# OPM/opm-autodiff

Measured on AMD Instinct MI355X. Metric: Newton iterations/sec, 1M-cell 3-phase black-oil (assembly + ILU0/BiCGStab solve + update), higher is better.
Workload: dtype f64

## Files before the change

### opm-autodiff_amd/csrc/internal.hpp

```cpp
#pragma once
#include <hip/hip_runtime.h>

#include <cstdarg>
#include <cstdio>
#include <cstdlib>
#include <cstring>
#include <memory>
#include <climits>
#include <string>
#include <type_traits>
#include <vector>

#include "../../include/opmhip.h"
#include "cpr_setup.hpp"

namespace opmhip {

constexpr int BS = 3;
constexpr int BB = 9;

#ifndef OPMHIP_TILE_ROWS
#define OPMHIP_TILE_ROWS 32
#endif
constexpr int TILE_ROWS = OPMHIP_TILE_ROWS;
// ... 285 lines not shown
    int ilu_fillin = 0;
    opmhip::Pattern pat;
    double *d_A = nullptr, *d_L = nullptr, *d_U = nullptr, *d_invD = nullptr;
    double *d_R = nullptr, *d_usum = nullptr;
    bool half_product = false;
    double *d_b = nullptr, *d_x = nullptr, *d_r = nullptr, *d_rw = nullptr, *d_p = nullptr, *d_v = nullptr,
           *d_s = nullptr, *d_t = nullptr, *d_pw = nullptr, *d_vu = nullptr;
    double *d_stageA = nullptr, *d_stageV = nullptr;
    double* d_scal = nullptr;
    double* d_part = nullptr;
    double minv_scale = 1.0;
    double* d_part2 = nullptr;
    int npart = 0;
    int last_solve_iterations = 0;
    int last_dot_count = 0;
    double* h_pinned = nullptr;
    static constexpr int RB_SLOTS = 4, RB_DOUBLES = 4;
    double* h_ring = nullptr;
    double* d_ring = nullptr;
    double rb_seq = 0.0;
    double rb_want[RB_SLOTS] = {0, 0, 0, 0};
    const double* d_done = nullptr;
    opmhip::WellsDev wells;
    opmhip::AsmDev asmb;
    opmhip::CommDev comm;
    opmhip::CprDev cpr;
    opmhip::Profiler prof;
    std::vector<void*> allocs;
    struct HostRange { const void* p; size_t bytes; };
    std::vector<HostRange> pinned;
// ... 136 lines not shown
    return slot;
}
inline void prof_span_end(opmhip_ctx* c, int slot, hipStream_t s = nullptr) {
    if (slot < 0) return;
    const int e = prof_event(c, s);
    if (e >= 0) c->prof.e1[slot] = e; else c->prof.cls[slot] = -1;
}

int build_pattern(opmhip_ctx* c, int Nb, int Nghost, int nnzb, const int* rows, const int* cols);

void launch_permute_blocks(opmhip_ctx* c, const double* nat, double* internal);
void launch_unpermute_blocks(opmhip_ctx* c, const double* internal, double* nat);
void launch_vec_to_internal(opmhip_ctx* c, const double* nat, double* internal, int cells = -1);
void launch_vec_to_natural(opmhip_ctx* c, const double* internal, double* nat, int cells = -1);
void launch_zero_diag_fix(opmhip_ctx* c);
int launch_spmv(opmhip_ctx* c, double* x, double* y, int ndot, const double* w0, double xs = 1.0, bool exchange = false, const double* uadd = nullptr, const double* w1 = nullptr);
bool half_product_wanted(const opmhip_ctx* c);
void launch_wells_residual(opmhip_ctx* c, const double* d_resWell, double* r);
void launch_wells_add_to_matrix(opmhip_ctx* c, int w0, int nw, int serial, const int* d_pair_ptr, const int* d_entry);
int launch_wells_recover(opmhip_ctx* c, const double* d_resWell, const double* x, double* d_xw);
void launch_ilu_factor(opmhip_ctx* c, bool fix_zero_diagonal = false, const FactorRider* rider = nullptr);
int cpr_factor_rider(opmhip_ctx* c, FactorRider* r);
void launch_ilu_apply(opmhip_ctx* c, const double* d, double* v, double w_override = -1.0, double* unscaled = nullptr, const double* addp = nullptr, double* work = nullptr, double* usum = nullptr);
int cpr_update(opmhip_ctx* c, bool solveBoundary = true);
void launch_cpr_apply(opmhip_ctx* c, const double* d, double* v);
int cpr_set_weights(opmhip_ctx* c, const double* w);
int cpr_level_sizes(const opmhip_ctx* c, int* n, int* nnz, int cap);
void cpr_shutdown(opmhip_ctx* c);
bool cpr_coarse_pivot_failed(opmhip_ctx* c);
int cpr_ilu_levels_in_force(const opmhip_ctx* c);
inline bool use_cpr(const opmhip_ctx* c) { return c->cfg.preconditioner == OPMHIP_PRECOND_CPR_QUASIIMPES || c->cfg.preconditioner == OPMHIP_PRECOND_CPR_TRUEIMPES; }
// ... 41 lines not shown
```

### opm-autodiff_amd/csrc/solver.hip

```cpp
#include <hip/hip_runtime.h>
#include <hip/hip_ext.h>
#include <atomic>

#include <chrono>
#include <cmath>
#include <cstdlib>

#include "internal.hpp"

namespace opmhip {

#ifndef OPMHIP_STAGE_DEPTH
#define OPMHIP_STAGE_DEPTH 16
#endif
typedef double v2d_t __attribute__((ext_vector_type(2)));
__device__ __forceinline__ double2 ld_stream(const double2* p) {
    const v2d_t t = __builtin_nontemporal_load(reinterpret_cast<const v2d_t*>(p));
    return make_double2(t.x, t.y);
}
__device__ __forceinline__ void st_rowsum(double* p, double v) {
    __builtin_nontemporal_store(v, p);
}
__device__ __forceinline__ void stage_doubles(const double* __restrict__ src, double* __restrict__ dst, int n, int lane) {
    const double2* __restrict__ s2 = reinterpret_cast<const double2*>(src);
// ... 267 lines not shown
                             const double* __restrict__ L, const double* __restrict__ U, const double* __restrict__ invD,
                             double* __restrict__ out) {
    const int p = blockIdx.x * blockDim.x + threadIdx.x;
    if (p >= Nb) return;
    int li = lrowptr[p], ui = urowptr[p];
    for (int k = rowptr[p]; k < rowptr[p + 1]; ++k) {
        if (col[k] >= Nb) {
            for (int q = 0; q < BB; ++q) out[(size_t)k * BB + q] = 0.0;
            continue;
        }
        const double* src = (col[k] < p) ? &L[(size_t)(li++) * BB] : (col[k] == p) ? &invD[(size_t)p * BB] : &U[(size_t)(ui++) * BB];
        for (int q = 0; q < BB; ++q) out[(size_t)k * BB + q] = src[q];
    }
}

template <int NDOT>
__global__ __launch_bounds__(64) void k_spmv(const int4* __restrict__ sched, const int* __restrict__ rowptr,
                                             const int* __restrict__ col, const double* __restrict__ val,
                                             const double* __restrict__ x, double* __restrict__ y,
                                             const double* __restrict__ w0, double* __restrict__ part, int npart,
                                             const double* __restrict__ done, double xs) {
    TILE_LDS
    const int lane = threadIdx.x, t = blockIdx.x;
    if (*done != 0.0) return;
    const int4 rows = sched[t];
    if (rows.y <= rows.x) {
        if (NDOT >= 1 && lane == 0) { part[t] = 0.0; if (NDOT == 2) part[npart + t] = 0.0; }
        return;
    }
    TileCtx T;
// ... 155 lines not shown
        __builtin_amdgcn_sched_barrier(0);
    }
    if (NDOT >= 1) {
        sd0 = wave_sum(sd0);
        if (NDOT == 2) sd1 = wave_sum(sd1);
        if (lane == 0) { part[blockIdx.x] = sd0; if (NDOT == 2) part[npart + blockIdx.x] = sd1; }
    }
}

template <int NDOT, bool UADD = false>
__global__ __launch_bounds__(64) void k_spmv_pipe_st(int npos, const int4* __restrict__ sched, const unsigned* __restrict__ stWord,
                                                     const unsigned char* __restrict__ stKoff, const int* __restrict__ stTable,
                                                     const double* __restrict__ val, const double* __restrict__ x, double* __restrict__ y,
                                                     const double* __restrict__ w0, double* __restrict__ part, int npart,
                                                     const double* __restrict__ done, double xs, const double* __restrict__ uadd = nullptr,
                                                     const double* __restrict__ w1 = nullptr) {
    TILE_LDS
    __shared__ int4 ssched[PIPE_MAX_STEPS];
    const int lane = threadIdx.x, G = gridDim.x;
    constexpr int U = 16;
    const int nsteps = ((int)blockIdx.x < npos) ? (npos - (int)blockIdx.x + G - 1) / G : 0;
    if (nsteps <= 0) {
        if (NDOT >= 1 && lane == 0) { part[blockIdx.x] = 0.0; if (NDOT >= 2) part[npart + blockIdx.x] = 0.0; if (NDOT == 3) part[2 * npart + blockIdx.x] = 0.0; }
        return;
    }
    const double stop = *done;
    for (int i = lane; i < nsteps; i += 64) ssched[i] = sched[(int)blockIdx.x + i * G];
    if (stop != 0.0) return;
    wave_sync();
    struct StW { unsigned w; int koff, tab; };
    struct StS {
        int k0e, n, n2;
        double2 tmp[U];
    };
    struct StM {
        int kb, nrow;
        double xx[PGCH][3];
        double ww[NDOT >= 1 ? 3 : 1];
// ... 97 lines not shown
                if (NDOT >= 2) { double d1 = acc[0] * acc[0]; d1 += acc[1] * acc[1]; d1 += acc[2] * acc[2]; sd1 += d1; }
                if constexpr (NDOT == 3) { double d2 = acc[0] * m.w2[0]; d2 += acc[1] * m.w2[1]; d2 += acc[2] * m.w2[2]; sd2 += d2; }
            }
        }
        wave_sync();
        __builtin_amdgcn_sched_barrier(0);
        stageGm(st + 1, wq, m);
        __builtin_amdgcn_sched_barrier(0);
        stageW(st + 2, wq);
        __builtin_amdgcn_sched_barrier(0);
    }
    if (NDOT >= 1) {
        sd0 = wave_sum(sd0);
        if (NDOT >= 2) sd1 = wave_sum(sd1);
        if (NDOT == 3) sd2 = wave_sum(sd2);
        if (lane == 0) { part[blockIdx.x] = sd0; if (NDOT >= 2) part[npart + blockIdx.x] = sd1; if (NDOT == 3) part[2 * npart + blockIdx.x] = sd2; }
    }
}

enum { SW_L = 0, SW_LF = 1, SW_UF = 2 };
template <int K> __device__ __forceinline__ double second_result(const double* __restrict__ addp, int r, double wout) {
    if (!addp) return wout;
    return (K == 1 ? addp[r] : 0.0) + wout;
}
template <int SHAPE>
__global__ __launch_bounds__(64) void k_ilu_sweep(int tile_begin, int ntc, int n0, int rhs_from_d, const int* __restrict__ tile_row0,
                                                  const int* __restrict__ prow, const int* __restrict__ pcol,
                                                  const double* __restrict__ P, const double* __restrict__ invD,
                                                  const double* __restrict__ d, double* __restrict__ vu, double* __restrict__ v,
                                                  const double* __restrict__ addp, int relax_mode, double w, const double* __restrict__ done) {
    TILE_LDS
// ... 844 lines not shown
                for (int k = 0; k < 4; ++k) s += Dw[i * 4 + k] * Bb[k * 3 + j];
                tmp[i][j] = s;
            }
        double* blk = &A[(size_t)entry[pair_ptr[w] + q] * BB];
        for (int i = 0; i < 3; ++i)
            for (int j = 0; j < 3; ++j) {
                double s = 0.0;
                for (int k = 0; k < 4; ++k) s += Cc[k * 3 + i] * tmp[k][j];
                blk[i * 3 + j] += -s;
            }
    }
}

constexpr int VB = 256;
constexpr int VPT = 8;
__device__ __forceinline__ void block_partials(double a, double b, double* part, int npart, int nsum) {
    __shared__ double sh[2][VB / 64];
    a = wave_sum(a);
    if (nsum > 1) b = wave_sum(b);
    const int lane = threadIdx.x & 63, wv = threadIdx.x >> 6;
    if (lane == 0) { sh[0][wv] = a; sh[1][wv] = b; }
    __syncthreads();
    if (threadIdx.x == 0) {
        double s = sh[0][0];
        for (int i = 1; i < VB / 64; ++i) s += sh[0][i];
        part[blockIdx.x] = s;
        if (nsum > 1) {
            double u = sh[1][0];
            for (int i = 1; i < VB / 64; ++i) u += sh[1][i];
            part[npart + blockIdx.x] = u;
        }
    }
}
__global__ __launch_bounds__(VB) void k_bicg_init(int n, const double* __restrict__ b, double* __restrict__ r,
                                                  double* __restrict__ rw, double* __restrict__ p, double* __restrict__ x,
                                                  double* __restrict__ v, double* __restrict__ part, int npart) {
    double s = 0.0;
    const int base = blockIdx.x * VB * VPT + threadIdx.x;
#pragma unroll
    for (int u = 0; u < VPT; ++u) {
        const int e = base + u * VB;
        if (e < n) {
            const double be = b[e];
            r[e] = be; rw[e] = be; p[e] = be; x[e] = 0.0; v[e] = 0.0;
            s += be * be;
        }
    }
    block_partials(s, 0.0, part, npart, 1);
}
__global__ __launch_bounds__(VB) void k_bicg_pupdate(int n, const double* __restrict__ scal, double* __restrict__ p,
                                                     const double* __restrict__ v, const double* __restrict__ r) {
    if (scal[SC_DONE] != 0.0) return;
    const double omega = scal[SC_OMEGA], beta = scal[SC_BETA];
    const int base = blockIdx.x * VB * VPT + threadIdx.x;
#pragma unroll
    for (int u = 0; u < VPT; ++u) {
        const int e = base + u * VB;
        if (e < n) p[e] = (p[e] - omega * __builtin_nontemporal_load(&v[e])) * beta + r[e];
    }
}
template <bool SR = false>
__global__ __launch_bounds__(VB) void k_bicg_upd1(int n, const double* __restrict__ scal, double* __restrict__ r,
                                                  const double* __restrict__ v, double* __restrict__ part, int npart, double half = -1.0) {
    if (scal[SC_DONE] != 0.0 && !(SR && scal[SC_DONEH] == half)) return;
    const double alpha = scal[SC_ALPHA];
    double s = 0.0;
    const int base = blockIdx.x * VB * VPT + threadIdx.x;
#pragma unroll
    for (int u = 0; u < VPT; ++u) {
        const int e = base + u * VB;
        if (e < n) {
            const double re = r[e] - alpha * __builtin_nontemporal_load(&v[e]);
            r[e] = re;
            s += re * re;
        }
    }
    if (!SR) block_partials(s, 0.0, part, npart, 1);
}
__global__ __launch_bounds__(VB) void k_bicg_xhalf(int n, const double* __restrict__ scal, double* __restrict__ x, const double* __restrict__ pw, double ws) {
    const double alpha = scal[SC_ALPHA];
    const int base = blockIdx.x * VB * VPT + threadIdx.x;
#pragma unroll
    for (int u = 0; u < VPT; ++u) {
        const int e = base + u * VB;
        if (e < n) x[e] += alpha * (ws * pw[e]);
    }
}
template <bool SR = false>
__global__ __launch_bounds__(VB) void k_bicg_upd2(int n, const double* __restrict__ scal, double* __restrict__ x,
                                                  const double* __restrict__ pw, const double* __restrict__ sv, double* __restrict__ r,
                                                  const double* __restrict__ tv, const double* __restrict__ rw,
                                                  double* __restrict__ part, int npart, double ws, double half = -1.0) {
    if (scal[SC_DONE] != 0.0 && !(SR && scal[SC_DONEH] == half)) return;
    const double alpha = scal[SC_ALPHA], omega = scal[SC_OMEGA];
    double s = 0.0, q = 0.0;
    const int base = blockIdx.x * VB * VPT + threadIdx.x;
#pragma unroll
    for (int u = 0; u < VPT; ++u) {
        const int e = base + u * VB;
        if (e < n) {
            const double xh = __builtin_nontemporal_load(&x[e]) + alpha * (ws * __builtin_nontemporal_load(&pw[e]));
            __builtin_nontemporal_store(xh + omega * (ws * __builtin_nontemporal_load(&sv[e])), &x[e]);
            const double re = r[e] - omega * __builtin_nontemporal_load(&tv[e]);
            r[e] = re;
            s += re * re;
            q += rw[e] * re;
        }
    }
    if (!SR) block_partials(s, q, part, npart, 2);
}
__global__ __launch_bounds__(VB) void k_dots(int n, const double* __restrict__ a, const double* __restrict__ b,
                                             double* __restrict__ part, int npart, int nsum) {
    double s = 0.0, q = 0.0;
    const int base = blockIdx.x * VB * VPT + threadIdx.x;
#pragma unroll
    for (int u = 0; u < VPT; ++u) {
        const int e = base + u * VB;
        if (e < n) { s += a[e] * b[e]; q += a[e] * a[e]; }
    }
    block_partials(s, q, part, npart, nsum);
}
__global__ __launch_bounds__(VB) void k_dots3(int n, const double* __restrict__ a, const double* __restrict__ b, const double* __restrict__ c3,
                                              double* __restrict__ part, int npart) {
    __shared__ double sh[3][VB / 64];
// ... 55 lines not shown
        case FIN_NORM_RHO: {
            scal[SC_NORM] = sqrt(s0);
            const double rhop = scal[SC_RHO];
            scal[SC_RHOP] = rhop; scal[SC_RHO] = s1;
            scal[SC_BETA] = (s1 / rhop) * (scal[SC_ALPHA] / scal[SC_OMEGA]);
        } break;
    }
    if (hslot && (mode == FIN_NORM || mode == FIN_NORM_RHO)) {
        const double norm = scal[SC_NORM], norm0 = scal[SC_NORM0];
        const double stop = (norm < tol * norm0) ? 1.0 : 0.0;
        scal[SC_DONE] = stop;
        hslot[0] = norm; hslot[1] = norm0; hslot[2] = stop;
        __hip_atomic_store(&hslot[3], seq, __ATOMIC_RELEASE, __HIP_MEMORY_SCOPE_SYSTEM);
    }
}
__device__ __forceinline__ void finalize_scalars3(int mode, double s0, double s1, double s2, double* __restrict__ scal, double tol, double* hslot, double seq, double half) {
    const double rr = scal[SC_RR];
    double rrn;
    if (mode == FIN_SR1) {
        const double rho = scal[SC_RHO];
        const double alpha = rho / s0;
        scal[SC_TMP1] = s0;
        scal[SC_ALPHA] = alpha;
        rrn = (rr - 2.0 * alpha * s2) + alpha * alpha * s1;
        scal[SC_RHOH] = rho - alpha * s0;
    } else {
        const double omega = s0 / s1;
        scal[SC_TMP1] = s0; scal[SC_TMP2] = s1;
        scal[SC_OMEGA] = omega;
        rrn = (rr - 2.0 * omega * s0) + omega * omega * s1;
// ... 51 lines not shown
    finalize_scalars3(mode, a, b, c3, scal, tol, hslot, seq, half);
}
__global__ __launch_bounds__(VB) void k_finalize(int mode, int count, const double* __restrict__ part, int npart,
                                                 double* __restrict__ scal, double tol, double* hslot, double seq) {
    __shared__ double sh[2][VB];
    constexpr int FU = 8;
    double va[FU], vb[FU];
#pragma unroll
    for (int u = 0; u < FU; ++u) {
        const int i = (int)threadIdx.x + u * VB;
        const int j = i < count ? i : 0;
        va[u] = part[j]; vb[u] = part[npart + j];
    }
    const double stop = (mode != FIN_INIT && mode != FIN_TRUE) ? scal[SC_DONE] : 0.0;
    if (stop != 0.0) {
        if (threadIdx.x == 0 && hslot && (mode == FIN_NORM || mode == FIN_NORM_RHO)) {
            hslot[0] = scal[SC_NORM]; hslot[1] = scal[SC_NORM0]; hslot[2] = 1.0;
            __hip_atomic_store(&hslot[3], seq, __ATOMIC_RELEASE, __HIP_MEMORY_SCOPE_SYSTEM);
        }
        return;
    }
    double a = 0.0, b = 0.0;
#pragma unroll
    for (int u = 0; u < FU; ++u)
        if ((int)threadIdx.x + u * VB < count) { a += va[u]; b += vb[u]; }
    for (int i = (int)threadIdx.x + FU * VB; i < count; i += VB) { a += part[i]; b += part[npart + i]; }
    sh[0][threadIdx.x] = a; sh[1][threadIdx.x] = b;
    __syncthreads();
    for (int o = VB / 2; o >= 64; o >>= 1) {
        if ((int)threadIdx.x < o) { sh[0][threadIdx.x] += sh[0][threadIdx.x + o]; sh[1][threadIdx.x] += sh[1][threadIdx.x + o]; }
        __syncthreads();
    }
    if (threadIdx.x >= 64) return;
    a = sh[0][threadIdx.x]; b = sh[1][threadIdx.x];
#pragma unroll
    for (int o = 32; o > 0; o >>= 1) { a += __shfl_down(a, o, 64); b += __shfl_down(b, o, 64); }
    if (threadIdx.x != 0) return;
    finalize_scalars(mode, a, b, scal, tol, hslot, seq);
}
static_assert(RED1_BLOCKS <= VB, "the last workgroup holds one slice sum per thread");
__global__ __launch_bounds__(VB) void k_reduce_finalize(int mode, int count, const double* __restrict__ part, int npart, double* out,
                                                        unsigned* ticket, double* __restrict__ scal, double tol, double* hslot, double seq) {
    __shared__ double sh[2][VB];
    __shared__ bool last;
    if (mode != FIN_INIT && mode != FIN_LOCAL && mode != FIN_TRUE && scal[SC_DONE] != 0.0) {
        if (blockIdx.x == 0 && threadIdx.x == 0 && hslot && (mode == FIN_NORM || mode == FIN_NORM_RHO)) {
            hslot[0] = scal[SC_NORM]; hslot[1] = scal[SC_NORM0]; hslot[2] = 1.0;
            __hip_atomic_store(&hslot[3], seq, __ATOMIC_RELEASE, __HIP_MEMORY_SCOPE_SYSTEM);
        }
        return;
    }
    const int chunk = (count + RED1_BLOCKS - 1) / RED1_BLOCKS;
    const int b0 = blockIdx.x * chunk, e0 = min(count, b0 + chunk);
    double a0 = 0.0, a1 = 0.0;
    for (int i = b0 + threadIdx.x; i < e0; i += VB) { a0 += part[i]; a1 += part[npart + i]; }
    sh[0][threadIdx.x] = a0; sh[1][threadIdx.x] = a1;
    __syncthreads();
    for (int o = VB / 2; o > 0; o >>= 1) {
        if ((int)threadIdx.x < o) { sh[0][threadIdx.x] += sh[0][threadIdx.x + o]; sh[1][threadIdx.x] += sh[1][threadIdx.x + o]; }
        __syncthreads();
    }
    if (threadIdx.x == 0) {
        __hip_atomic_store(&out[blockIdx.x], sh[0][0], __ATOMIC_RELAXED, __HIP_MEMORY_SCOPE_AGENT);
        __hip_atomic_store(&out[RED1_BLOCKS + blockIdx.x], sh[1][0], __ATOMIC_RELAXED, __HIP_MEMORY_SCOPE_AGENT);
// ... 107 lines not shown
    const int w = spmv_pipe_wgs(c);
    return c->pat.maxRowBlocks <= PGCH && w > 0 && c->pat.tiles.nsched > w;
}
bool half_product_wanted(const opmhip_ctx* c) {
    const Pattern& P = c->pat;
    if (!P.rest.on || c->cfg.half_product < 0 || use_cpr(c)) return false;
    if (c->cfg.half_product > 0) return true;
    return spmv_pipelined(c);
}
static bool spmv_dots_env() {
    static const bool v = [] { const char* e = tuning_env("OPMHIP_DOTS_SEPARATE"); return e && std::atoi(e) != 0; }();
    return v;
}
static bool spmv_dots_separate(const opmhip_ctx* c) { return c->wells.any() || spmv_dots_env(); }
static int launch_spmv_part(opmhip_ctx* c, int p0, int np, const double* x, double* y, int ndot, const double* w0, double xs, int pofs, int cls,
                            const double* uadd = nullptr, const double* w1 = nullptr) {
    const Pattern& P = c->pat;
    if (np <= 0) return 0;
    double* part = c->d_part + pofs;
    int es = -1, ee = -1;
    const bool timed = prof_kernel_scope(c, cls, &es, &ee);
    hipEvent_t e0 = timed ? c->prof.ev[es] : nullptr, e1 = timed ? c->prof.ev[ee] : nullptr;
    if (uadd) {
        const RestSched& R = P.rest;
        const int4* rsched = reinterpret_cast<const int4*>(R.d_sched) + p0;
        const int pipeWgs = std::max(8, spmv_pipe_wgs(c));
        const int steps = std::min((np + pipeWgs - 1) / pipeWgs, PIPE_MAX_STEPS);
        const int grid = 8 * (((np + steps - 1) / steps + 7) / 8);
        const int* tab = R.d_table + (size_t)p0 * 16;
        if (ndot == 0)
            hipExtLaunchKernelGGL((k_spmv_pipe_st<0, true>), dim3(grid), dim3(64), 0, c->stream, e0, e1, 0, np, rsched, R.d_word, R.d_koff, tab, c->d_R, x, y, w0, part, c->npart, c->d_done, xs, uadd, (const double*)nullptr);
        else if (ndot == 1)
            hipExtLaunchKernelGGL((k_spmv_pipe_st<1, true>), dim3(grid), dim3(64), 0, c->stream, e0, e1, 0, np, rsched, R.d_word, R.d_koff, tab, c->d_R, x, y, w0, part, c->npart, c->d_done, xs, uadd, (const double*)nullptr);
        else if (ndot == 2)
            hipExtLaunchKernelGGL((k_spmv_pipe_st<2, true>), dim3(grid), dim3(64), 0, c->stream, e0, e1, 0, np, rsched, R.d_word, R.d_koff, tab, c->d_R, x, y, w0, part, c->npart, c->d_done, xs, uadd, (const double*)nullptr);
        else
            hipExtLaunchKernelGGL((k_spmv_pipe_st<3, true>), dim3(grid), dim3(64), 0, c->stream, e0, e1, 0, np, rsched, R.d_word, R.d_koff, tab, c->d_R, x, y, w0, part, c->npart, c->d_done, xs, uadd, w1);
        return ndot > 0 ? grid : 0;
    }
    const int4* sched = reinterpret_cast<const int4*>(P.tiles.d_spmvSched) + p0;
    if (spmv_pipelined(c)) {
        const int pipeWgs = spmv_pipe_wgs(c);
        const int steps = std::min((np + pipeWgs - 1) / pipeWgs, PIPE_MAX_STEPS);
        const int grid = 8 * (((np + steps - 1) / steps + 7) / 8);
        const bool inInt = p0 < P.tiles.nschedInt, inBnd = p0 + np > P.tiles.nschedInt;
        if ((!inInt || P.tiles.stencilPart[0]) && (!inBnd || P.tiles.stencilPart[1])) {
            const StencilForm& S = P.tiles.st;
            const int* tab = S.d_table + (size_t)p0 * 16;
            if (ndot == 0)
                hipExtLaunchKernelGGL((k_spmv_pipe_st<0, false>), dim3(grid), dim3(64), 0, c->stream, e0, e1, 0, np, sched, S.d_word, S.d_koff, tab, c->d_A, x, y, w0, part, c->npart, c->d_done, xs, (const double*)nullptr, (const double*)nullptr);
            else if (ndot == 1)
                hipExtLaunchKernelGGL((k_spmv_pipe_st<1, false>), dim3(grid), dim3(64), 0, c->stream, e0, e1, 0, np, sched, S.d_word, S.d_koff, tab, c->d_A, x, y, w0, part, c->npart, c->d_done, xs, (const double*)nullptr, (const double*)nullptr);
            else if (ndot == 2)
                hipExtLaunchKernelGGL((k_spmv_pipe_st<2, false>), dim3(grid), dim3(64), 0, c->stream, e0, e1, 0, np, sched, S.d_word, S.d_koff, tab, c->d_A, x, y, w0, part, c->npart, c->d_done, xs, (const double*)nullptr, (const double*)nullptr);
            else
                hipExtLaunchKernelGGL((k_spmv_pipe_st<3, false>), dim3(grid), dim3(64), 0, c->stream, e0, e1, 0, np, sched, S.d_word, S.d_koff, tab, c->d_A, x, y, w0, part, c->npart, c->d_done, xs, (const double*)nullptr, w1);
            return ndot > 0 ? grid : 0;
        }
        if (ndot == 0)
            hipExtLaunchKernelGGL(k_spmv_pipe<0>, dim3(grid), dim3(64), 0, c->stream, e0, e1, 0, np, sched, P.d_rowptr, P.d_col, c->d_A, x, y, w0, part, c->npart, c->d_done, xs);
        else if (ndot == 1)
            hipExtLaunchKernelGGL(k_spmv_pipe<1>, dim3(grid), dim3(64), 0, c->stream, e0, e1, 0, np, sched, P.d_rowptr, P.d_col, c->d_A, x, y, w0, part, c->npart, c->d_done, xs);
        else
            hipExtLaunchKernelGGL(k_spmv_pipe<2>, dim3(grid), dim3(64), 0, c->stream, e0, e1, 0, np, sched, P.d_rowptr, P.d_col, c->d_A, x, y, w0, part, c->npart, c->d_done, xs);
        return ndot > 0 ? grid : 0;
    }
    if (ndot == 0)
        hipExtLaunchKernelGGL(k_spmv<0>, dim3(np), dim3(64), 0, c->stream, e0, e1, 0, sched, P.d_rowptr, P.d_col, c->d_A, x, y, w0, part, c->npart, c->d_done, xs);
    else if (ndot == 1)
        hipExtLaunchKernelGGL(k_spmv<1>, dim3(np), dim3(64), 0, c->stream, e0, e1, 0, sched, P.d_rowptr, P.d_col, c->d_A, x, y, w0, part, c->npart, c->d_done, xs);
    else
// ... 4 lines not shown
    WellsDev& W = c->wells;
    const size_t n = (size_t)c->pat.Nb * BS;
    launch_vec_to_natural(c, x, c->d_stageV);
    OPMHIP_HIP(c, hipMemcpyAsync(W.h_x, c->d_stageV, n * sizeof(double), hipMemcpyDeviceToHost, c->stream));
    launch_vec_to_natural(c, y, c->d_stageV);
    OPMHIP_HIP(c, hipMemcpyAsync(W.h_y, c->d_stageV, n * sizeof(double), hipMemcpyDeviceToHost, c->stream));
    OPMHIP_HIP(c, hipStreamSynchronize(c->stream));
    if (xs != 1.0)
        for (size_t i = 0; i < n; ++i) W.h_x[i] *= xs;
    W.ms_apply(W.ms_user, W.h_x, W.h_y);
    OPMHIP_HIP(c, hipMemcpyAsync(c->d_stageV, W.h_y, n * sizeof(double), hipMemcpyHostToDevice, c->stream));
    launch_vec_to_internal(c, c->d_stageV, y);
    OPMHIP_HIP(c, hipStreamSynchronize(c->stream));
    return OPMHIP_SUCCESS;
}
int launch_spmv(opmhip_ctx* c, double* x, double* y, int ndot, const double* w0, double xs, bool exchange, const double* uadd, const double* w1) {
    const Pattern& P = c->pat;
    const bool wells = c->wells.num_wells > 0;
    const bool bndPlain = uadd && P.Nghost > 0 && P.tiles.nsched > P.tiles.nschedInt;
    const bool plain3 = spmv_pipelined(c);
    const bool rides3 = uadd ? (!bndPlain || (plain3 && P.tiles.stencilPart[1]))
                             : (plain3 && P.tiles.stencilPart[0] && (P.tiles.nsched == P.tiles.nschedInt || P.tiles.stencilPart[1]));
    const int fused = (spmv_dots_separate(c) || (ndot == 3 && !rides3)) ? 0 : ndot;
    const bool halo = exchange && c->comm.halo_set && c->comm.nneigh > 0;
    if (exchange && !halo && c->comm.nranks > 1) comm_halo_bystander(c);
    const int nInt = uadd ? P.rest.nschedInt : P.tiles.nschedInt;
    const int bnd0 = (uadd && !bndPlain) ? P.rest.nschedInt : P.tiles.nschedInt;
    const int nBnd = (uadd && !bndPlain) ? P.rest.nsched - P.rest.nschedInt : P.tiles.nsched - P.tiles.nschedInt;
    const double* uBnd = bndPlain ? nullptr : uadd;
    int rc, cnt = 0;
    if (halo && nBnd > 0) {
        if ((rc = comm_halo_begin(c, x))) return rc;
        cnt += launch_spmv_part(c, 0, nInt, x, y, fused, w0, xs, cnt, PROF_SPMV, uadd, w1);
        if ((rc = comm_halo_end(c))) return rc;
        cnt += launch_spmv_part(c, bnd0, nBnd, x, y, fused, w0, xs, cnt, PROF_SPMV_BOUNDARY, uBnd, w1);
    } else {
        if (halo && (rc = comm_halo_f64(c, x, BS))) return rc;
        cnt += launch_spmv_part(c, 0, nInt, x, y, fused, w0, xs, cnt, PROF_SPMV, uadd, w1);
        if (nBnd > 0) cnt += launch_spmv_part(c, bnd0, nBnd, x, y, fused, w0, xs, cnt, bndPlain ? PROF_SPMV_BOUNDARY : PROF_SPMV, uBnd, w1);
    }
    if (c->wells.num_ms > 0 && (rc = ms_wells_apply(c, x, y, xs))) return rc;
    if (wells && (rc = launch_wells_apply(c, x, y, xs))) return rc;
    if (fused == 0 && ndot > 0) {
        const int n = P.Nb * BS;
        const int ps = prof_begin(c, PROF_VECTOR);
        if (ndot == 3) {
            cnt = std::min(vec_blocks(n), RED1_SINGLE_MAX);
            hipLaunchKernelGGL(k_dots3, dim3(cnt), dim3(VB), 0, c->stream, n, y, w0, w1, c->d_part, c->npart);
        } else {
            hipLaunchKernelGGL(k_dots, dim3(vec_blocks(n)), dim3(VB), 0, c->stream, n, y, w0, c->d_part, c->npart, ndot);
            cnt = vec_blocks(n);
        }
        prof_end(c, ps);
// ... 110 lines not shown
        if (col < C - 1)
            hipLaunchKernelGGL(k_ilu_sweep<SW_L>, grid(nt), dim3(64), 0, c->stream, tb, nt, n0, 0, T.d_row0, P.d_lrowptr, P.d_lcol, c->d_L,
                               c->d_invD, d, vu, v, addp, mode, w, c->d_done);
        else
            hipLaunchKernelGGL(k_ilu_sweep<SW_LF>, grid(nt), dim3(64), 0, c->stream, tb, nt, n0, 0, T.d_row0, P.d_lrowptr, P.d_lcol, c->d_L,
                               c->d_invD, d, vu, v, addp, mode, w, c->d_done);
    }
    for (int col = (C > 1 ? C - 2 : 0); col >= 0; --col) {
        const int tb = T.colorTile[col], nt = T.colorTile[col + 1] - tb;
        if (nt <= 0) continue;
        hipLaunchKernelGGL(k_ilu_sweep<SW_UF>, grid(nt), dim3(64), 0, c->stream, tb, nt, 0, col == 0 ? 1 : 0, T.d_row0, P.d_urowptr, P.d_ucol,
                           c->d_U, c->d_invD, d, vu, v, addp, mode, w, c->d_done);
    }
    prof_end(c, ps);
}
static int finalize(opmhip_ctx* c, int mode, int count, int rb_half = -1) {
    const double tol = c->cfg.tolerance;
    double* hslot = nullptr;
    double seq = 0.0;
    if (rb_half >= 0) {
        const int sl = rb_half % opmhip_ctx::RB_SLOTS;
        hslot = c->d_ring + (size_t)sl * opmhip_ctx::RB_DOUBLES;
        seq = (c->rb_seq += 1.0);
        c->rb_want[sl] = seq;
    }
    if (c->comm.nranks > 1) {
        const int span = prof_span_begin(c, PROF_ALLREDUCE);
        if (count > RED1_SINGLE_MAX)
            hipLaunchKernelGGL(k_reduce_finalize, dim3(RED1_BLOCKS), dim3(VB), 0, c->stream, (int)FIN_LOCAL, count, c->d_part, c->npart, c->d_part2,
                               reinterpret_cast<unsigned*>(c->d_part2 + 2 * RED1_BLOCKS), c->comm.d_red, tol, (double*)nullptr, 0.0);
        else
            hipLaunchKernelGGL(k_local_sums, dim3(1), dim3(VB), 0, c->stream, count, c->d_part, c->npart, c->comm.d_red);
        c->comm.reduce_span_open = true;
        const int rc = comm_allreduce(c, c->comm.d_red, 2, 0);
        c->comm.reduce_span_open = false;
        prof_span_end(c, span);
        if (rc) return rc;
        hipLaunchKernelGGL(k_finalize, dim3(1), dim3(VB), 0, c->stream, mode, 1, c->comm.d_red, 1, c->d_scal, tol, hslot, seq);
        return OPMHIP_SUCCESS;
    }
// ... 34 lines not shown
    (void)finalize(c, FIN_NORM_RHO, nb);
}

static int read_scalars(opmhip_ctx* c) {
    OPMHIP_HIP(c, hipMemcpyAsync(c->h_pinned, c->d_scal, SC_COUNT * sizeof(double), hipMemcpyDeviceToHost, c->stream));
    OPMHIP_HIP(c, hipStreamSynchronize(c->stream));
    return OPMHIP_SUCCESS;
}
enum { HALF_ALL = 0, HALF_PRECOND = 1, HALF_REST = 2 };
static int enqueue_half(opmhip_ctx* c, int h, int part = HALF_ALL) {
    const Pattern& P = c->pat;
    const int n = P.Nb * BS, nb = vec_blocks(n);
    const bool cpr = use_cpr(c);
    const bool hp = !cpr && c->half_product;
    const bool sr = c->cfg.fused_reductions > 0;
    const bool precTalks = cpr && c->cpr.gather.on;
    const bool head = part != HALF_REST, rest = part != HALF_PRECOND;
    const bool applyNow = part == HALF_ALL || (precTalks ? part == HALF_REST : part == HALF_PRECOND);
    int rc, ps;
    if ((h & 1) == 0) {
        if (head && h > 0) {
            ps = prof_begin(c, PROF_VECTOR);
            hipLaunchKernelGGL(k_bicg_pupdate, dim3(nb), dim3(VB), 0, c->stream, n, c->d_scal, c->d_p, c->d_v, c->d_r);
            prof_end(c, ps);
        }
        if (applyNow) {
            if (cpr) launch_cpr_apply(c, c->d_p, c->d_pw);
            else launch_ilu_apply(c, c->d_p, c->d_pw, -1.0, &c->minv_scale, nullptr, nullptr, hp ? c->d_usum : nullptr);
            if (cpr && c->cpr.apply_rc) { rc = c->cpr.apply_rc; c->cpr.apply_rc = 0; return rc; }
        }
        if (!rest) return OPMHIP_SUCCESS;
        if (sr) {
            if ((rc = launch_spmv(c, c->d_pw, c->d_v, 3, c->d_rw, c->minv_scale, true, hp ? c->d_usum : nullptr, c->d_r))) return rc;
            ps = prof_begin(c, PROF_VECTOR);
            if ((rc = finalize3(c, FIN_SR1, dot_count(c), h))) return rc;
            hipLaunchKernelGGL(k_bicg_upd1<true>, dim3(nb), dim3(VB), 0, c->stream, n, c->d_scal, c->d_r, c->d_v, c->d_part, c->npart, (double)h);
            prof_end(c, ps);
            return OPMHIP_SUCCESS;
        }
        if ((rc = launch_spmv(c, c->d_pw, c->d_v, 1, c->d_rw, c->minv_scale, true, hp ? c->d_usum : nullptr))) return rc;
        ps = prof_begin(c, PROF_VECTOR);
        if ((rc = finalize(c, FIN_ALPHA, dot_count(c)))) return rc;
        hipLaunchKernelGGL(k_bicg_upd1<false>, dim3(nb), dim3(VB), 0, c->stream, n, c->d_scal, c->d_r, c->d_v, c->d_part, c->npart, -1.0);
        if ((rc = finalize(c, FIN_NORM, nb, h))) return rc;
        prof_end(c, ps);
    } else {
        if (applyNow) {
            if (cpr) launch_cpr_apply(c, c->d_r, c->d_s);
            else launch_ilu_apply(c, c->d_r, c->d_s, -1.0, &c->minv_scale, nullptr, nullptr, hp ? c->d_usum : nullptr);
            if (cpr && c->cpr.apply_rc) { rc = c->cpr.apply_rc; c->cpr.apply_rc = 0; return rc; }
        }
        if (!rest) return OPMHIP_SUCCESS;
        if (sr) {
            if ((rc = launch_spmv(c, c->d_s, c->d_t, 3, c->d_r, c->minv_scale, true, hp ? c->d_usum : nullptr, c->d_rw))) return rc;
            ps = prof_begin(c, PROF_VECTOR);
            if ((rc = finalize3(c, FIN_SR2, dot_count(c), h))) return rc;
            hipLaunchKernelGGL(k_bicg_upd2<true>, dim3(nb), dim3(VB), 0, c->stream, n, c->d_scal, c->d_x, c->d_pw, c->d_s, c->d_r, c->d_t, c->d_rw, c->d_part, c->npart, c->minv_scale, (double)h);
            prof_end(c, ps);
            return OPMHIP_SUCCESS;
        }
        if ((rc = launch_spmv(c, c->d_s, c->d_t, 2, c->d_r, c->minv_scale, true, hp ? c->d_usum : nullptr))) return rc;
        ps = prof_begin(c, PROF_VECTOR);
        if ((rc = finalize(c, FIN_OMEGA, dot_count(c)))) return rc;
        hipLaunchKernelGGL(k_bicg_upd2<false>, dim3(nb), dim3(VB), 0, c->stream, n, c->d_scal, c->d_x, c->d_pw, c->d_s, c->d_r, c->d_t, c->d_rw, c->d_part, c->npart, c->minv_scale, -1.0);
        if ((rc = finalize(c, FIN_NORM_RHO, nb, h))) return rc;
        prof_end(c, ps);
    }
    return OPMHIP_SUCCESS;
}
static int wait_half(opmhip_ctx* c, int h, double* norm, double* norm_0) {
    const int sl = h % opmhip_ctx::RB_SLOTS;
    const volatile double* slot = c->h_ring + (size_t)sl * opmhip_ctx::RB_DOUBLES;
    const double want = c->rb_want[sl];
    const auto t0 = std::chrono::steady_clock::now();
    for (unsigned long spin = 1;; ++spin) {
        if (slot[3] == want) break;
        if ((spin & 0xFFFFu) == 0) {
            const hipError_t e = hipStreamQuery(c->stream);
            if (e == hipSuccess) {
                if (slot[3] == want) break;
// ... 89 lines not shown
```

Baseline: 81.23.

## Fold BiCGStab scalar finalize into last-block of SpMV and update kernels

Adds a last-workgroup ticket scheme so the final block of the SpMV dot-product kernel and the vector-update kernels reduces the per-block partials and computes the BiCGStab scalars (alpha, omega, norm/rho) itself. This removes separate finalize kernel launches from each half iteration, cutting launch count and serialization on the stream. In exchange it adds agent-scope atomic stores, a global ticket counter, and a serial single-wave reduction at the tail of each kernel. It only runs on single-rank, half-product, non-fused-reduction paths without wells or boundary rows, and an environment variable can turn it off.

```diff
diff --git a/opm-autodiff_amd/csrc/internal.hpp b/opm-autodiff_amd/csrc/internal.hpp
--- a/opm-autodiff_amd/csrc/internal.hpp
+++ b/opm-autodiff_amd/csrc/internal.hpp
@@ -323,6 +323,7 @@
     int npart = 0;
     int last_solve_iterations = 0;
     int last_dot_count = 0;
+    bool last_dots_folded = false;
     double* h_pinned = nullptr;
     static constexpr int RB_SLOTS = 4, RB_DOUBLES = 4;
     double* h_ring = nullptr;
@@ -489,7 +490,9 @@
 void launch_vec_to_internal(opmhip_ctx* c, const double* nat, double* internal, int cells = -1);
 void launch_vec_to_natural(opmhip_ctx* c, const double* internal, double* nat, int cells = -1);
 void launch_zero_diag_fix(opmhip_ctx* c);
-int launch_spmv(opmhip_ctx* c, double* x, double* y, int ndot, const double* w0, double xs = 1.0, bool exchange = false, const double* uadd = nullptr, const double* w1 = nullptr);
+struct FinFold;
+int launch_spmv(opmhip_ctx* c, double* x, double* y, int ndot, const double* w0, double xs = 1.0, bool exchange = false, const double* uadd = nullptr, const double* w1 = nullptr,
+                const FinFold* fin = nullptr);
 bool half_product_wanted(const opmhip_ctx* c);
 void launch_wells_residual(opmhip_ctx* c, const double* d_resWell, double* r);
 void launch_wells_add_to_matrix(opmhip_ctx* c, int w0, int nw, int serial, const int* d_pair_ptr, const int* d_entry);
diff --git a/opm-autodiff_amd/csrc/solver.hip b/opm-autodiff_amd/csrc/solver.hip
--- a/opm-autodiff_amd/csrc/solver.hip
+++ b/opm-autodiff_amd/csrc/solver.hip
@@ -305,6 +305,18 @@
     }
 }
 
+struct FinFold {
+    unsigned* ticket = nullptr;
+    double* scal = nullptr;
+    double* hslot = nullptr;
+    double tol = 0.0, seq = 0.0;
+    int mode = 0;
+};
+__device__ __forceinline__ void fin_store(double* p, double v, bool agent);
+__device__ __forceinline__ bool fin_ticket(unsigned* ticket);
+template <int NS> __device__ __forceinline__ void fin_fold_wave(const FinFold& f, int count, const double* part, int npart);
+__device__ __forceinline__ void fin_answer_stopped(int mode, const double* scal, double* hslot, double seq);
+
 template <int NDOT>
 __global__ __launch_bounds__(64) void k_spmv(const int4* __restrict__ sched, const int* __restrict__ rowptr,
                                              const int* __restrict__ col, const double* __restrict__ val,
@@ -490,14 +502,26 @@
                                                      const double* __restrict__ val, const double* __restrict__ x, double* __restrict__ y,
                                                      const double* __restrict__ w0, double* __restrict__ part, int npart,
                                                      const double* __restrict__ done, double xs, const double* __restrict__ uadd = nullptr,
-                                                     const double* __restrict__ w1 = nullptr) {
+                                                     const double* __restrict__ w1 = nullptr, FinFold fin = FinFold()) {
     TILE_LDS
     __shared__ int4 ssched[PIPE_MAX_STEPS];
     const int lane = threadIdx.x, G = gridDim.x;
     constexpr int U = 16;
+    const bool fold = NDOT >= 1 && NDOT <= 2 && fin.ticket;
+    auto leave = [&](double s0, double s1, double s2) {
+        bool last = false;
+        if (lane == 0) {
+            fin_store(&part[blockIdx.x], s0, fold);
+            if (NDOT >= 2) fin_store(&part[npart + blockIdx.x], s1, fold);
+            if (NDOT == 3) part[2 * npart + blockIdx.x] = s2;
+            if (fold) last = fin_ticket(fin.ticket);
+        }
+        if (fold && __shfl((int)last, 0, 64)) fin_fold_wave<NDOT >= 2 ? 2 : 1>(fin, G, part, npart);
+    };
     const int nsteps = ((int)blockIdx.x < npos) ? (npos - (int)blockIdx.x + G - 1) / G : 0;
     if (nsteps <= 0) {
-        if (NDOT >= 1 && lane == 0) { part[blockIdx.x] = 0.0; if (NDOT >= 2) part[npart + blockIdx.x] = 0.0; if (NDOT == 3) part[2 * npart + blockIdx.x] = 0.0; }
+        if (fold && *done != 0.0) return;
+        if (NDOT >= 1) leave(0.0, 0.0, 0.0);
         return;
     }
     const double stop = *done;
@@ -625,7 +649,7 @@
         sd0 = wave_sum(sd0);
         if (NDOT >= 2) sd1 = wave_sum(sd1);
         if (NDOT == 3) sd2 = wave_sum(sd2);
-        if (lane == 0) { part[blockIdx.x] = sd0; if (NDOT >= 2) part[npart + blockIdx.x] = sd1; if (NDOT == 3) part[2 * npart + blockIdx.x] = sd2; }
+        leave(sd0, sd1, sd2);
     }
 }
 
@@ -1500,8 +1524,10 @@
 
 constexpr int VB = 256;
 constexpr int VPT = 8;
-__device__ __forceinline__ void block_partials(double a, double b, double* part, int npart, int nsum) {
+__device__ __forceinline__ void block_partials(double a, double b, double* part, int npart, int nsum, const FinFold& fin = FinFold()) {
     __shared__ double sh[2][VB / 64];
+    __shared__ int lastWg;
+    const bool fold = fin.ticket != nullptr;
     a = wave_sum(a);
     if (nsum > 1) b = wave_sum(b);
     const int lane = threadIdx.x & 63, wv = threadIdx.x >> 6;
@@ -1510,13 +1536,19 @@
     if (threadIdx.x == 0) {
         double s = sh[0][0];
         for (int i = 1; i < VB / 64; ++i) s += sh[0][i];
-        part[blockIdx.x] = s;
+        fin_store(&part[blockIdx.x], s, fold);
         if (nsum > 1) {
             double u = sh[1][0];
             for (int i = 1; i < VB / 64; ++i) u += sh[1][i];
-            part[npart + blockIdx.x] = u;
-        }
-    }
+            fin_store(&part[npart + blockIdx.x], u, fold);
+        }
+        if (fold) lastWg = fin_ticket(fin.ticket);
+    }
+    if (!fold) return;
+    __syncthreads();
+    if (!lastWg || threadIdx.x >= 64) return;
+    if (nsum > 1) fin_fold_wave<2>(fin, gridDim.x, part, npart);
+    else fin_fold_wave<1>(fin, gridDim.x, part, npart);
 }
 __global__ __launch_bounds__(VB) void k_bicg_init(int n, const double* __restrict__ b, double* __restrict__ r,
                                                   double* __restrict__ rw, double* __restrict__ p, double* __restrict__ x,
@@ -1546,9 +1578,13 @@
     }
 }
 template <bool SR = false>
-__global__ __launch_bounds__(VB) void k_bicg_upd1(int n, const double* __restrict__ scal, double* __restrict__ r,
-                                                  const double* __restrict__ v, double* __restrict__ part, int npart, double half = -1.0) {
-    if (scal[SC_DONE] != 0.0 && !(SR && scal[SC_DONEH] == half)) return;
+__global__ __launch_bounds__(VB) void k_bicg_upd1(int n, const double* scal, double* __restrict__ r,
+                                                  const double* __restrict__ v, double* __restrict__ part, int npart, double half = -1.0,
+                                                  FinFold fin = FinFold()) {
+    if (scal[SC_DONE] != 0.0 && !(SR && scal[SC_DONEH] == half)) {
+        if (fin.ticket && blockIdx.x == 0 && threadIdx.x == 0) fin_answer_stopped(fin.mode, scal, fin.hslot, fin.seq);
+        return;
+    }
     const double alpha = scal[SC_ALPHA];
     double s = 0.0;
     const int base = blockIdx.x * VB * VPT + threadIdx.x;
@@ -1561,7 +1597,7 @@
             s += re * re;
         }
     }
-    if (!SR) block_partials(s, 0.0, part, npart, 1);
+    if (!SR) block_partials(s, 0.0, part, npart, 1, fin);
 }
 __global__ __launch_bounds__(VB) void k_bicg_xhalf(int n, const double* __restrict__ scal, double* __restrict__ x, const double* __restrict__ pw, double ws) {
     const double alpha = scal[SC_ALPHA];
@@ -1573,11 +1609,14 @@
     }
 }
 template <bool SR = false>
-__global__ __launch_bounds__(VB) void k_bicg_upd2(int n, const double* __restrict__ scal, double* __restrict__ x,
+__global__ __launch_bounds__(VB) void k_bicg_upd2(int n, const double* scal, double* __restrict__ x,
                                                   const double* __restrict__ pw, const double* __restrict__ sv, double* __restrict__ r,
                                                   const double* __restrict__ tv, const double* __restrict__ rw,
-                                                  double* __restrict__ part, int npart, double ws, double half = -1.0) {
-    if (scal[SC_DONE] != 0.0 && !(SR && scal[SC_DONEH] == half)) return;
+                                                  double* __restrict__ part, int npart, double ws, double half = -1.0, FinFold fin = FinFold()) {
+    if (scal[SC_DONE] != 0.0 && !(SR && scal[SC_DONEH] == half)) {
+        if (fin.ticket && blockIdx.x == 0 && threadIdx.x == 0) fin_answer_stopped(fin.mode, scal, fin.hslot, fin.seq);
+        return;
+    }
     const double alpha = scal[SC_ALPHA], omega = scal[SC_OMEGA];
     double s = 0.0, q = 0.0;
     const int base = blockIdx.x * VB * VPT + threadIdx.x;
@@ -1593,7 +1632,7 @@
             q += rw[e] * re;
         }
     }
-    if (!SR) block_partials(s, q, part, npart, 2);
+    if (!SR) block_partials(s, q, part, npart, 2, fin);
 }
 __global__ __launch_bounds__(VB) void k_dots(int n, const double* __restrict__ a, const double* __restrict__ b,
                                              double* __restrict__ part, int npart, int nsum) {
@@ -1679,6 +1718,61 @@
         __hip_atomic_store(&hslot[3], seq, __ATOMIC_RELEASE, __HIP_MEMORY_SCOPE_SYSTEM);
     }
 }
+__device__ __forceinline__ void fin_answer_stopped(int mode, const double* scal, double* hslot, double seq) {
+    if (hslot && (mode == FIN_NORM || mode == FIN_NORM_RHO)) {
+        hslot[0] = scal[SC_NORM]; hslot[1] = scal[SC_NORM0]; hslot[2] = 1.0;
+        __hip_atomic_store(&hslot[3], seq, __ATOMIC_RELEASE, __HIP_MEMORY_SCOPE_SYSTEM);
+    }
+}
+__device__ __forceinline__ void fin_store(double* p, double v, bool agent) {
+    if (agent) __hip_atomic_store(p, v, __ATOMIC_RELAXED, __HIP_MEMORY_SCOPE_AGENT);
+    else *p = v;
+}
+__device__ __forceinline__ bool fin_ticket(unsigned* ticket) {
+    asm volatile("s_waitcnt vmcnt(0)" ::: "memory");
+    const bool last = __hip_atomic_fetch_add(ticket, 1u, __ATOMIC_RELAXED, __HIP_MEMORY_SCOPE_AGENT) == gridDim.x - 1;
+    if (last) __hip_atomic_store(ticket, 0u, __ATOMIC_RELAXED, __HIP_MEMORY_SCOPE_AGENT);
+    return last;
+}
+template <int NS>
+__device__ __forceinline__ void fin_fold_wave(const FinFold& f, int count, const double* part, int npart) {
+    static_assert(VB == 256, "four k_finalize threads per lane");
+    __builtin_amdgcn_fence(__ATOMIC_ACQUIRE, "wavefront");
+    const int l = threadIdx.x & 63;
+    constexpr int FU = 8;
+    double s[NS][4];
+#pragma unroll
+    for (int k = 0; k < NS; ++k)
+#pragma unroll
+        for (int q = 0; q < 4; ++q) s[k][q] = 0.0;
+    for (int base = 0; base < count; base += FU * VB) {
+        double v[NS][FU][4];
+#pragma unroll
+        for (int u = 0; u < FU; ++u)
+#pragma unroll
+            for (int q = 0; q < 4; ++q) {
+                const int i = base + u * VB + q * 64 + l, j = i < count ? i : 0;
+#pragma unroll
+                for (int k = 0; k < NS; ++k) v[k][u][q] = __hip_atomic_load(&part[(size_t)k * npart + j], __ATOMIC_RELAXED, __HIP_MEMORY_SCOPE_AGENT);
+            }
+#pragma unroll
+        for (int u = 0; u < FU; ++u)
+#pragma unroll
+            for (int q = 0; q < 4; ++q)
+                if (base + u * VB + q * 64 + l < count) {
+#pragma unroll
+                    for (int k = 0; k < NS; ++k) s[k][q] += v[k][u][q];
+                }
+    }
+    double a[2] = {0.0, 0.0};
+#pragma unroll
+    for (int k = 0; k < NS; ++k) {
+        a[k] = (s[k][0] + s[k][2]) + (s[k][1] + s[k][3]);
+#pragma unroll
+        for (int o = 32; o > 0; o >>= 1) a[k] += __shfl_down(a[k], o, 64);
+    }
+    if (l == 0) finalize_scalars(f.mode, a[0], a[1], f.scal, f.tol, f.hslot, f.seq);
+}
 __device__ __forceinline__ void finalize_scalars3(int mode, double s0, double s1, double s2, double* __restrict__ scal, double tol, double* hslot, double seq, double half) {
     const double rr = scal[SC_RR];
     double rrn;
@@ -1760,10 +1854,7 @@
     }
     const double stop = (mode != FIN_INIT && mode != FIN_TRUE) ? scal[SC_DONE] : 0.0;
     if (stop != 0.0) {
-        if (threadIdx.x == 0 && hslot && (mode == FIN_NORM || mode == FIN_NORM_RHO)) {
-            hslot[0] = scal[SC_NORM]; hslot[1] = scal[SC_NORM0]; hslot[2] = 1.0;
-            __hip_atomic_store(&hslot[3], seq, __ATOMIC_RELEASE, __HIP_MEMORY_SCOPE_SYSTEM);
-        }
+        if (threadIdx.x == 0) fin_answer_stopped(mode, scal, hslot, seq);
         return;
     }
     double a = 0.0, b = 0.0;
@@ -1790,10 +1881,7 @@
     __shared__ double sh[2][VB];
     __shared__ bool last;
     if (mode != FIN_INIT && mode != FIN_LOCAL && mode != FIN_TRUE && scal[SC_DONE] != 0.0) {
-        if (blockIdx.x == 0 && threadIdx.x == 0 && hslot && (mode == FIN_NORM || mode == FIN_NORM_RHO)) {
-            hslot[0] = scal[SC_NORM]; hslot[1] = scal[SC_NORM0]; hslot[2] = 1.0;
-            __hip_atomic_store(&hslot[3], seq, __ATOMIC_RELEASE, __HIP_MEMORY_SCOPE_SYSTEM);
-        }
+        if (blockIdx.x == 0 && threadIdx.x == 0) fin_answer_stopped(mode, scal, hslot, seq);
         return;
     }
     const int chunk = (count + RED1_BLOCKS - 1) / RED1_BLOCKS;
@@ -1931,7 +2019,7 @@
 }
 static bool spmv_dots_separate(const opmhip_ctx* c) { return c->wells.any() || spmv_dots_env(); }
 static int launch_spmv_part(opmhip_ctx* c, int p0, int np, const double* x, double* y, int ndot, const double* w0, double xs, int pofs, int cls,
-                            const double* uadd = nullptr, const double* w1 = nullptr) {
+                            const double* uadd = nullptr, const double* w1 = nullptr, const FinFold* fin = nullptr) {
     const Pattern& P = c->pat;
     if (np <= 0) return 0;
     double* part = c->d_part + pofs;
@@ -1945,14 +2033,16 @@
         const int steps = std::min((np + pipeWgs - 1) / pipeWgs, PIPE_MAX_STEPS);
         const int grid = 8 * (((np + steps - 1) / steps + 7) / 8);
         const int* tab = R.d_table + (size_t)p0 * 16;
+        FinFold f;
+        if (fin && pofs == 0 && (ndot == 1 || ndot == 2) && grid <= RED1_SINGLE_MAX) { f = *fin; c->last_dots_folded = true; }
         if (ndot == 0)
-            hipExtLaunchKernelGGL((k_spmv_pipe_st<0, true>), dim3(grid), dim3(64), 0, c->stream, e0, e1, 0, np, rsched, R.d_word, R.d_koff, tab, c->d_R, x, y, w0, part, c->npart, c->d_done, xs, uadd, (const double*)nullptr);
+            hipExtLaunchKernelGGL((k_spmv_pipe_st<0, true>), dim3(grid), dim3(64), 0, c->stream, e0, e1, 0, np, rsched, R.d_word, R.d_koff, tab, c->d_R, x, y, w0, part, c->npart, c->d_done, xs, uadd, (const double*)nullptr, FinFold());
         else if (ndot == 1)
-            hipExtLaunchKernelGGL((k_spmv_pipe_st<1, true>), dim3(grid), dim3(64), 0, c->stream, e0, e1, 0, np, rsched, R.d_word, R.d_koff, tab, c->d_R, x, y, w0, part, c->npart, c->d_done, xs, uadd, (const double*)nullptr);
+            hipExtLaunchKernelGGL((k_spmv_pipe_st<1, true>), dim3(grid), dim3(64), 0, c->stream, e0, e1, 0, np, rsched, R.d_word, R.d_koff, tab, c->d_R, x, y, w0, part, c->npart, c->d_done, xs, uadd, (const double*)nullptr, f);
         else if (ndot == 2)
-            hipExtLaunchKernelGGL((k_spmv_pipe_st<2, true>), dim3(grid), dim3(64), 0, c->stream, e0, e1, 0, np, rsched, R.d_word, R.d_koff, tab, c->d_R, x, y, w0, part, c->npart, c->d_done, xs, uadd, (const double*)nullptr);
+            hipExtLaunchKernelGGL((k_spmv_pipe_st<2, true>), dim3(grid), dim3(64), 0, c->stream, e0, e1, 0, np, rsched, R.d_word, R.d_koff, tab, c->d_R, x, y, w0, part, c->npart, c->d_done, xs, uadd, (const double*)nullptr, f);
         else
-            hipExtLaunchKernelGGL((k_spmv_pipe_st<3, true>), dim3(grid), dim3(64), 0, c->stream, e0, e1, 0, np, rsched, R.d_word, R.d_koff, tab, c->d_R, x, y, w0, part, c->npart, c->d_done, xs, uadd, w1);
+            hipExtLaunchKernelGGL((k_spmv_pipe_st<3, true>), dim3(grid), dim3(64), 0, c->stream, e0, e1, 0, np, rsched, R.d_word, R.d_koff, tab, c->d_R, x, y, w0, part, c->npart, c->d_done, xs, uadd, w1, FinFold());
         return ndot > 0 ? grid : 0;
     }
     const int4* sched = reinterpret_cast<const int4*>(P.tiles.d_spmvSched) + p0;
@@ -1965,13 +2055,13 @@
             const StencilForm& S = P.tiles.st;
             const int* tab = S.d_table + (size_t)p0 * 16;
             if (ndot == 0)
-                hipExtLaunchKernelGGL((k_spmv_pipe_st<0, false>), dim3(grid), dim3(64), 0, c->stream, e0, e1, 0, np, sched, S.d_word, S.d_koff, tab, c->d_A, x, y, w0, part, c->npart, c->d_done, xs, (const double*)nullptr, (const double*)nullptr);
+                hipExtLaunchKernelGGL((k_spmv_pipe_st<0, false>), dim3(grid), dim3(64), 0, c->stream, e0, e1, 0, np, sched, S.d_word, S.d_koff, tab, c->d_A, x, y, w0, part, c->npart, c->d_done, xs, (const double*)nullptr, (const double*)nullptr, FinFold());
             else if (ndot == 1)
-                hipExtLaunchKernelGGL((k_spmv_pipe_st<1, false>), dim3(grid), dim3(64), 0, c->stream, e0, e1, 0, np, sched, S.d_word, S.d_koff, tab, c->d_A, x, y, w0, part, c->npart, c->d_done, xs, (const double*)nullptr, (const double*)nullptr);
+                hipExtLaunchKernelGGL((k_spmv_pipe_st<1, false>), dim3(grid), dim3(64), 0, c->stream, e0, e1, 0, np, sched, S.d_word, S.d_koff, tab, c->d_A, x, y, w0, part, c->npart, c->d_done, xs, (const double*)nullptr, (const double*)nullptr, FinFold());
             else if (ndot == 2)
-                hipExtLaunchKernelGGL((k_spmv_pipe_st<2, false>), dim3(grid), dim3(64), 0, c->stream, e0, e1, 0, np, sched, S.d_word, S.d_koff, tab, c->d_A, x, y, w0, part, c->npart, c->d_done, xs, (const double*)nullptr, (const double*)nullptr);
+                hipExtLaunchKernelGGL((k_spmv_pipe_st<2, false>), dim3(grid), dim3(64), 0, c->stream, e0, e1, 0, np, sched, S.d_word, S.d_koff, tab, c->d_A, x, y, w0, part, c->npart, c->d_done, xs, (const double*)nullptr, (const double*)nullptr, FinFold());
             else
-                hipExtLaunchKernelGGL((k_spmv_pipe_st<3, false>), dim3(grid), dim3(64), 0, c->stream, e0, e1, 0, np, sched, S.d_word, S.d_koff, tab, c->d_A, x, y, w0, part, c->npart, c->d_done, xs, (const double*)nullptr, w1);
+                hipExtLaunchKernelGGL((k_spmv_pipe_st<3, false>), dim3(grid), dim3(64), 0, c->stream, e0, e1, 0, np, sched, S.d_word, S.d_koff, tab, c->d_A, x, y, w0, part, c->npart, c->d_done, xs, (const double*)nullptr, w1, FinFold());
             return ndot > 0 ? grid : 0;
         }
         if (ndot == 0)
@@ -2006,7 +2096,8 @@
     OPMHIP_HIP(c, hipStreamSynchronize(c->stream));
     return OPMHIP_SUCCESS;
 }
-int launch_spmv(opmhip_ctx* c, double* x, double* y, int ndot, const double* w0, double xs, bool exchange, const double* uadd, const double* w1) {
+int launch_spmv(opmhip_ctx* c, double* x, double* y, int ndot, const double* w0, double xs, bool exchange, const double* uadd, const double* w1,
+                const FinFold* fin) {
     const Pattern& P = c->pat;
     const bool wells = c->wells.num_wells > 0;
     const bool bndPlain = uadd && P.Nghost > 0 && P.tiles.nsched > P.tiles.nschedInt;
@@ -2021,6 +2112,8 @@
     const int nBnd = (uadd && !bndPlain) ? P.rest.nsched - P.rest.nschedInt : P.tiles.nsched - P.tiles.nschedInt;
     const double* uBnd = bndPlain ? nullptr : uadd;
     int rc, cnt = 0;
+    c->last_dots_folded = false;
+    if (fin && (c->comm.nranks > 1 || !uadd || fused != ndot || nBnd > 0 || wells || c->wells.num_ms > 0)) fin = nullptr;
     if (halo && nBnd > 0) {
         if ((rc = comm_halo_begin(c, x))) return rc;
         cnt += launch_spmv_part(c, 0, nInt, x, y, fused, w0, xs, cnt, PROF_SPMV, uadd, w1);
@@ -2028,7 +2121,7 @@
         cnt += launch_spmv_part(c, bnd0, nBnd, x, y, fused, w0, xs, cnt, PROF_SPMV_BOUNDARY, uBnd, w1);
     } else {
         if (halo && (rc = comm_halo_f64(c, x, BS))) return rc;
-        cnt += launch_spmv_part(c, 0, nInt, x, y, fused, w0, xs, cnt, PROF_SPMV, uadd, w1);
+        cnt += launch_spmv_part(c, 0, nInt, x, y, fused, w0, xs, cnt, PROF_SPMV, uadd, w1, fin);
         if (nBnd > 0) cnt += launch_spmv_part(c, bnd0, nBnd, x, y, fused, w0, xs, cnt, bndPlain ? PROF_SPMV_BOUNDARY : PROF_SPMV, uBnd, w1);
     }
     if (c->wells.num_ms > 0 && (rc = ms_wells_apply(c, x, y, xs))) return rc;
@@ -2169,16 +2262,37 @@
     }
     prof_end(c, ps);
 }
+static void ring_slot(opmhip_ctx* c, int rb_half, double** hslot, double* seq) {
+    *hslot = nullptr;
+    *seq = 0.0;
+    if (rb_half < 0) return;
+    const int sl = rb_half % opmhip_ctx::RB_SLOTS;
+    *hslot = c->d_ring + (size_t)sl * opmhip_ctx::RB_DOUBLES;
+    *seq = (c->rb_seq += 1.0);
+    c->rb_want[sl] = *seq;
+}
+static bool finalize_separate_env() {
+    static const bool v = [] { const char* e = tuning_env("OPMHIP_FINALIZE_SEPARATE"); return e && std::atoi(e) != 0; }();
+    return v;
+}
+static bool fold_scalar_stage(const opmhip_ctx* c, bool hp, bool sr) {
+    return hp && !sr && c->comm.nranks == 1 && !finalize_separate_env();
+}
+static_assert(2 * RED1_BLOCKS + 16 + 1 <= 1024, "d_part2 holds the slice sums, k_reduce_finalize's ticket and FinFold's");
+static FinFold fin_fold(opmhip_ctx* c, int mode, int rb_half = -1) {
+    FinFold f;
+    f.ticket = reinterpret_cast<unsigned*>(c->d_part2 + 2 * RED1_BLOCKS + 16);
+    f.scal = c->d_scal;
+    f.tol = c->cfg.tolerance;
+    f.mode = mode;
+    ring_slot(c, rb_half, &f.hslot, &f.seq);
+    return f;
+}
 static int finalize(opmhip_ctx* c, int mode, int count, int rb_half = -1) {
     const double tol = c->cfg.tolerance;
-    double* hslot = nullptr;
-    double seq = 0.0;
-    if (rb_half >= 0) {
-        const int sl = rb_half % opmhip_ctx::RB_SLOTS;
-        hslot = c->d_ring + (size_t)sl * opmhip_ctx::RB_DOUBLES;
-        seq = (c->rb_seq += 1.0);
-        c->rb_want[sl] = seq;
-    }
+    double* hslot;
+    double seq;
+    ring_slot(c, rb_half, &hslot, &seq);
     if (c->comm.nranks > 1) {
         const int span = prof_span_begin(c, PROF_ALLREDUCE);
         if (count > RED1_SINGLE_MAX)
@@ -2243,6 +2357,7 @@
     const bool cpr = use_cpr(c);
     const bool hp = !cpr && c->half_product;
     const bool sr = c->cfg.fused_reductions > 0;
+    const bool fold = fold_scalar_stage(c, hp, sr);
     const bool precTalks = cpr && c->cpr.gather.on;
     const bool head = part != HALF_REST, rest = part != HALF_PRECOND;
     const bool applyNow = part == HALF_ALL || (precTalks ? part == HALF_REST : part == HALF_PRECOND);
@@ -2267,11 +2382,16 @@
             prof_end(c, ps);
             return OPMHIP_SUCCESS;
         }
-        if ((rc = launch_spmv(c, c->d_pw, c->d_v, 1, c->d_rw, c->minv_scale, true, hp ? c->d_usum : nullptr))) return rc;
+        const FinFold fa = fin_fold(c, FIN_ALPHA);
+        if ((rc = launch_spmv(c, c->d_pw, c->d_v, 1, c->d_rw, c->minv_scale, true, hp ? c->d_usum : nullptr, nullptr, fold ? &fa : nullptr))) return rc;
         ps = prof_begin(c, PROF_VECTOR);
-        if ((rc = finalize(c, FIN_ALPHA, dot_count(c)))) return rc;
-        hipLaunchKernelGGL(k_bicg_upd1<false>, dim3(nb), dim3(VB), 0, c->stream, n, c->d_scal, c->d_r, c->d_v, c->d_part, c->npart, -1.0);
-        if ((rc = finalize(c, FIN_NORM, nb, h))) return rc;
+        if (!c->last_dots_folded && (rc = finalize(c, FIN_ALPHA, dot_count(c)))) return rc;
+        if (fold && nb <= RED1_SINGLE_MAX) {
+            hipLaunchKernelGGL(k_bicg_upd1<false>, dim3(nb), dim3(VB), 0, c->stream, n, c->d_scal, c->d_r, c->d_v, c->d_part, c->npart, -1.0, fin_fold(c, FIN_NORM, h));
+        } else {
+            hipLaunchKernelGGL(k_bicg_upd1<false>, dim3(nb), dim3(VB), 0, c->stream, n, c->d_scal, c->d_r, c->d_v, c->d_part, c->npart, -1.0, FinFold());
+            if ((rc = finalize(c, FIN_NORM, nb, h))) return rc;
+        }
         prof_end(c, ps);
     } else {
         if (applyNow) {
@@ -2288,11 +2408,18 @@
             prof_end(c, ps);
             return OPMHIP_SUCCESS;
         }
-        if ((rc = launch_spmv(c, c->d_s, c->d_t, 2, c->d_r, c->minv_scale, true, hp ? c->d_usum : nullptr))) return rc;
+        const FinFold fo = fin_fold(c, FIN_OMEGA);
+        if ((rc = launch_spmv(c, c->d_s, c->d_t, 2, c->d_r, c->minv_scale, true, hp ? c->d_usum : nullptr, nullptr, fold ? &fo : nullptr))) return rc;
         ps = prof_begin(c, PROF_VECTOR);
-        if ((rc = finalize(c, FIN_OMEGA, dot_count(c)))) return rc;
-        hipLaunchKernelGGL(k_bicg_upd2<false>, dim3(nb), dim3(VB), 0, c->stream, n, c->d_scal, c->d_x, c->d_pw, c->d_s, c->d_r, c->d_t, c->d_rw, c->d_part, c->npart, c->minv_scale, -1.0);
-        if ((rc = finalize(c, FIN_NORM_RHO, nb, h))) return rc;
+        if (!c->last_dots_folded && (rc = finalize(c, FIN_OMEGA, dot_count(c)))) return rc;
+        if (fold && nb <= RED1_SINGLE_MAX) {
+            hipLaunchKernelGGL(k_bicg_upd2<false>, dim3(nb), dim3(VB), 0, c->stream, n, c->d_scal, c->d_x, c->d_pw, c->d_s, c->d_r, c->d_t, c->d_rw, c->d_part, c->npart,
+                               c->minv_scale, -1.0, fin_fold(c, FIN_NORM_RHO, h));
+        } else {
+            hipLaunchKernelGGL(k_bicg_upd2<false>, dim3(nb), dim3(VB), 0, c->stream, n, c->d_scal, c->d_x, c->d_pw, c->d_s, c->d_r, c->d_t, c->d_rw, c->d_part, c->npart,
+                               c->minv_scale, -1.0, FinFold());
+            if ((rc = finalize(c, FIN_NORM_RHO, nb, h))) return rc;
+        }
         prof_end(c, ps);
     }
     return OPMHIP_SUCCESS;
```

New measurement: 77.31 (median of 2 runs). 0.952x the previous value.
